# tobiashepp/torch-mednet

Hardware: AMD Instinct MI355X
Metric: 128^3 patches/sec training, 3D U-Net 32-base-ch (higher is better)
Workload: dtype bf16; 1 GPU; ResidualUNet3D f_maps=[32, 64, 128, 256] 4-class, 128^3 patches, batch 4/GPU, fwd+DiceLoss+bwd+allreduce+Adam (BASELINE config 2); global_batch=4, parallelism=dp1, graph_replay=False, gradient_exchange=none (1 rank)

## Files before the change

include/mednet_hip.h:

```cpp
#ifndef MEDNET_HIP_H
#define MEDNET_HIP_H
#include <stddef.h>
#include <stdint.h>
#ifdef __cplusplus
extern "C" {
#endif

typedef void* mednet_stream;

enum { MEDNET_F32 = 0, MEDNET_BF16 = 1,
       MEDNET_F16 = 2,
       MEDNET_U8 = 3,
       MEDNET_I64 = 4   };
enum { MEDNET_NDHWC = 0, MEDNET_NCDHW = 1 };
enum { MEDNET_ACT_NONE = 0, MEDNET_ACT_RELU = 1, MEDNET_ACT_LEAKY = 2, MEDNET_ACT_ELU = 3 };
enum { MEDNET_POOL_MAX = 0, MEDNET_POOL_AVG = 1 };
enum { MEDNET_ALGO_AUTO = 0, MEDNET_ALGO_DIRECT = 1, MEDNET_ALGO_MFMA = 2, MEDNET_ALGO_EXACT = 3,
       MEDNET_ALGO_EXACT_BIT = 4,
       MEDNET_ALGO_SPLITW_BIT = 8 };
enum { MEDNET_PACK_LOW = 0x100,
       MEDNET_PACK_HIGH_ONLY = 0x200 };
enum { MEDNET_REG_L2 = 0, MEDNET_REG_L1 = 1 };
enum { MEDNET_CLASS_DICE = 0, MEDNET_CLASS_CE = 1, MEDNET_CLASS_DICE_CE = 2 };
enum {
// ... 56 lines not shown
int mednet_conv3d_wgrad_c1_gn(const void* x, const void* dz, const void* y, const float* coef, const float* bcoef, float* dw,
                              int n, int d, int h, int w, int cout, int act, int x_dtype, int dtype, void* ws, size_t ws_bytes,
                              mednet_stream stream);
int mednet_conv3d_wgrad_cm_gn_supported(int cin, int cout, int x_dtype, int dtype);
int mednet_conv3d_wgrad_cm_plan(int n, int d, int h, int w, int cin, int cout, int dtype, int gn, int* out4);
int mednet_conv3d_wgrad_cm_gn(const void* x, int x_layout, const void* dz, const void* y, const float* coef, const float* bcoef,
                              float* dw, int n, int d, int h, int w, int cin, int cout, int act, int x_dtype, int dtype, void* ws,
                              size_t ws_bytes, mednet_stream stream);
int mednet_conv3d_wgrad(const void* x, const void* dy, float* dw, float* dbias, int n, int d, int h, int w,
                        int cin, int cout, int ksize, int x_dtype, int x_layout, int dy_dtype, int dy_layout,
                        int algo, int workgroups, void* ws, size_t ws_bytes, mednet_stream stream);

int mednet_convt3d_fwd(const void* x, const void* packed, const float* bias, const void* skip, void* y, int n,
                       int d, int h, int w, int cin, int cout, int x_dtype, int y_dtype, int algo,
                       mednet_stream stream);
int mednet_convt3d_dgrad(const void* dy, const void* packed, void* dx, int n, int d, int h, int w, int cin,
                         int cout, int dy_dtype, int dx_dtype, int algo, mednet_stream stream);
size_t mednet_convt3d_wgrad_ws_bytes(int n, int d, int h, int w, int cin, int cout, int workgroups);
int mednet_convt3d_wgrad(const void* x, const void* dy, float* dw, float* dbias, int n, int d, int h, int w,
                         int cin, int cout, int x_dtype, int dy_dtype, int algo, int workgroups, void* ws,
                         size_t ws_bytes, mednet_stream stream);

size_t mednet_gn_ws_bytes(int n, int c, size_t spatial);
int mednet_gn_stats(const void* x, const float* gamma, const float* beta, float* stats, float* coef, int n,
                    size_t spatial, int c, int groups, float eps, int dtype, void* ws, size_t ws_bytes,
                    mednet_stream stream);
int mednet_gn_finalize(const float* partial, int chunks, const float* gamma, const float* beta, float* stats,
                       float* coef, int n, size_t spatial, int c, int groups, float eps, void* ws, size_t ws_bytes,
                       mednet_stream stream);
int mednet_gn_act_fwd(const void* x, const float* coef, const void* residual, void* z, int n, size_t spatial,
// ... 253 lines not shown
```

torch-mednet_amd/csrc/api.hip:

```cpp
#include <stdarg.h>
#include <string.h>
#include "common.h"
#include "conv.h"

static thread_local char g_err[512] = "";

int mednet_internal_fail(int code, const char* fmt, ...) {
  va_list ap;
  va_start(ap, fmt);
  vsnprintf(g_err, sizeof(g_err), fmt, ap);
  va_end(ap);
  return code;
}
int mednet_internal_check_launch(const char* what) {
  const hipError_t e = hipGetLastError();
  if (e != hipSuccess) return mednet_internal_fail(MEDNET_E_HIP, "%s: %s", what, hipGetErrorString(e));
  return MEDNET_OK;
}

struct Option {
  char name[32];
  int value;
};
static Option g_options[48];
// ... 636 lines not shown
    return fail(MEDNET_E_UNSUPPORTED, "convt3d_fwd: MFMA path does not take cin=%d cout=%d", cin, cout);
  if (mfma_ok && algo_base(algo) != MEDNET_ALGO_DIRECT)
    return ELT_CALL(x_dtype, launch_convt_fwd_mfma, x, pack_mfma(packed, L, 0), bias, skip, y, n, d, h, w, cin, cout,
                    (hipStream_t)stream, algo_lo_delta(algo, x_dtype, L));
  if (f32_mode) {
    if (algo_x3(algo) && L.mfma_bytes && conv_x3_supported(cin, cout, 3))
      return launch_convt_fwd_x3(x, pack_mfma(packed, L, 0), L.lo_delta, bias, skip, y, n, d, h, w, cin, cout, (hipStream_t)stream);
    return launch_convt_fwd_f32_mfma(x, pack_f32(packed, L, 0), bias, skip, y, n, d, h, w, cin, cout, (hipStream_t)stream);
  }
  ConvGeom g;
  g.n = n; g.od = 2 * d; g.oh = 2 * h; g.ow = 2 * w; g.id = d; g.ih = h; g.iw = w;
  g.k = cin; g.m = cout; g.ks = 3; g.in_planar = 0; g.out_planar = 0;
  return launch_direct<MAP_CT_FWD>(x, pack_f32(packed, L, 0), bias, skip, y, g, x_dtype, y_dtype, (hipStream_t)stream);
}

extern "C" int mednet_convt3d_dgrad(const void* dy, const void* packed, void* dx, int n, int d, int h, int w, int cin,
                                    int cout, int dy_dtype, int dx_dtype, int algo, mednet_stream stream) {
  int rc = conv_common_checks("convt3d_dgrad", n, d, h, w, cin, cout, 3, dy_dtype, dx_dtype);
  if (rc) return rc;
  const PackLayout L = pack_layout(cin, cout, 3);
  const bool mfma_ok = L.mfma_bytes && cin % 32 == 0 && cout % 32 == 0 && is16(dy_dtype) && dx_dtype == dy_dtype &&
                       conv_mfma_fits(n, 2 * d, 2 * h, 2 * w, cout);
  const bool f32_mode = algo_f32_mode(algo, dy_dtype, dx_dtype);
  if (algo_base(algo) == MEDNET_ALGO_MFMA && !mfma_ok && !f32_mode)
    return fail(MEDNET_E_UNSUPPORTED, "convt3d_dgrad: MFMA path does not take cin=%d cout=%d", cin, cout);
  if (mfma_ok && algo_base(algo) != MEDNET_ALGO_DIRECT)
    return ELT_CALL(dy_dtype, launch_convt_dgrad_mfma, dy, pack_mfma(packed, L, 1), dx, n, d, h, w, cin, cout,
                    (hipStream_t)stream, algo_lo_delta(algo, dy_dtype, L));
  if (f32_mode) {
    if (algo_x3(algo) && L.mfma_bytes && conv_x3_supported(cin, cout, 3) && conv_x3_fits(2 * d, 2 * h, 2 * w, cout))
// ... 66 lines not shown
```

torch-mednet_amd/csrc/conv_mfma.hip:

```cpp
#include <type_traits>
#include "conv.h"

#include "elt16.inc"

namespace mednet {

template <int KIND>
struct FwdTile;
template <>
struct FwdTile<1> {
  static constexpr int TZ = 4, TY = 8, TX = 16, STRIDE = 1;
};
template <>
struct FwdTile<2> {
  static constexpr int TZ = 2, TY = 4, TX = 16, STRIDE = 2;
};
template <>
struct FwdTile<3> {
  static constexpr int TZ = 4, TY = 8, TX = 8, STRIDE = 1;
};
static bool narrow_bricks(int w) {
  const int mode = tuning_option("conv_narrow", 1);
  return mode != 0 && (w <= 8 || (mode == 2 && (w + 7) / 8 < 2 * ((w + 15) / 16)));
}
// ... 1024 lines not shown
      if (oz < od && oy < oh && ox < ow) {
        const size_t o = ((((size_t)n * od + oz) * oh + oy) * ow + ox) * a.cout + cb * 32 + piece * 8;
        const eltx8 sk = skr[it];
        eltx8 ov;
#pragma unroll
        for (int j = 0; j < 4; ++j) {
          ov[j] = (elt)(lo[j] + (float)sk[j]);
          ov[4 + j] = (elt)(hi[j] + (float)sk[4 + j]);
        }
        *reinterpret_cast<eltx8*>(a.y + o) = ov;
      }
    }
  }
}

int launch_convt_fwd_mfma(const void* x, const void* sec, const float* bias, const void* skip, void* y, int n, int d,
                          int h, int w, int cin, int cout, hipStream_t s, size_t lo_delta) {
  constexpr size_t lds = 512 * 32 * 4;
  static_assert(lds >= ((size_t)2 * 3 * 5 * 17 + 27 * 2 * 32) * 16 && lds <= 80 * 1024, "LDS plan of convt_fwd");
  CtArgs a;
  a.x = (const elt*)x;
  a.wpk = (const elt*)sec;
  a.bias = bias;
  a.skip = (const elt*)skip;
  a.y = (elt*)y;
  a.n = n; a.id = d; a.ih = h; a.iw = w; a.cin = cin; a.cout = cout;
  a.tiles_z = (d + 1) / 2;
  a.tiles_y = (h + 3) / 4;
  a.tiles_x = (w + 15) / 16;
  a.ntiles = n * a.tiles_z * a.tiles_y * a.tiles_x;
  a.nkc_in = cin / 16;
  a.nkc = lo_delta ? 2 * a.nkc_in : a.nkc_in;
// ... 412 lines not shown
  GnbSpec g;
  g.y = gn_y;
  g.z = gn_z;
  g.act = gn_act;
  return launch_fwd<2>(dy, packed_section, dx, n, d, h, w, 2 * d, 2 * h, 2 * w, cout, cin, gn_partial, s, MEDNET_ACT_NONE, nullptr, g,
                       nullptr, lo_delta);
}

struct Wg2Args {
  const elt* A;
  const elt* B;
  float* part;
  int n, d, h, w, ka, kb;
  int tiles_z, tiles_y, tiles_x, ntiles;
  int nab, nbb, splits;
  unsigned rcp_tiles_x, rcp_tiles_y, rcp_tiles_z;
  unsigned bytesA, bytesB;
};

template <int TX>
__global__ __launch_bounds__(512, 2) void wgrad_mfma2_kernel(Wg2Args a) {
  constexpr int TZ = 4, TY = 8, HZ = TZ + 2, HY = TY + 2, HX = TX + 2;
  static_assert(TX == 16 || TX == 8, "brick widths");
  constexpr int NA = TZ * TY * TX, NB = HZ * HY * HX;
  constexpr int A_ROUNDS = NA * 4 / 512, B_ROUNDS = (NB * 4 + 511) / 512;
  constexpr int KSTEPS = NA / 16;
  typedef __attribute__((ext_vector_type(4))) unsigned u32x4;
  extern __shared__ __attribute__((aligned(16))) char smem[];
  elt* A_lds = reinterpret_cast<elt*>(smem);
  elt* B_lds = reinterpret_cast<elt*>(smem) + NA * 32;
// ... 60 lines not shown
  };

  f32x16 acc[7];
#pragma unroll
  for (int i = 0; i < 7; ++i)
#pragma unroll
    for (int j = 0; j < 16; ++j) acc[i][j] = 0.f;
  const char* Ab = reinterpret_cast<const char*>(A_lds) + coloff;
  const char* Bb = reinterpret_cast<const char*>(B_lds) + coloff;
  int toff[7];
#pragma unroll
  for (int i = 0; i < 7; ++i) {
    const int tap = tw + 4 * i < 27 ? tw + 4 * i : 26;
    toff[i] = (((tap / 9) * HY + (tap / 3) % 3) * HX + tap % 3) * 64;
  }

  int tile = split;
  const int t_step = a.splits, t_end = a.ntiles;
  if (tile < t_end) {
    const Next first = plan_next(tile, true);
#pragma unroll
    for (int j = 0; j < A_ROUNDS + B_ROUNDS; ++j) fetch_one(j, first);
  }
  static_assert(A_ROUNDS + B_ROUNDS <= KSTEPS / 2, "one staging load per k-step");
  for (; tile < t_end; tile += t_step) {
    __syncthreads();
    commit();
    __syncthreads();
    const Next nx = plan_next(tile + t_step, tile + t_step < t_end);
#pragma unroll
    for (int k2 = 0; k2 < KSTEPS / 2; ++k2) {
      const int ks = 2 * k2 + kgrp;
      const eltx8 fa = tr_operand(Ab + (ks * 16 + 8 * hk + q) * 64, 4 * 64);
      const int krow = TX == 16 ? ks : 2 * ks;
      const char* brow = Bb + (((krow / TY) * HY + krow % TY) * HX + (TX == 16 ? 8 * hk : hk * HX) + q) * 64;
      eltx8 fb[7];
#pragma unroll
      for (int i = 0; i < 7; ++i) fb[i] = tr_operand(brow + toff[i], 4 * 64);
      if (k2 < A_ROUNDS + B_ROUNDS) fetch_one(k2, nx);
#pragma unroll
      for (int i = 0; i < 7; ++i) acc[i] = MEDNET_MFMA_32x32x16(fa, fb[i], acc[i], 0, 0, 0);
    }
  }
  float* mlds = reinterpret_cast<float*>(smem);
#pragma unroll
  for (int i0 = 0; i0 < 7; i0 += 4) {
    __syncthreads();
    if (kgrp == 1) {
#pragma unroll
      for (int i = i0; i < (i0 + 4 < 7 ? i0 + 4 : 7); ++i)
#pragma unroll
        for (int j = 0; j < 16; ++j) mlds[((tw * 4 + (i - i0)) * 16 + j) * 64 + lane] = acc[i][j];
    }
    __syncthreads();
    if (kgrp == 0) {
#pragma unroll
// ... 20 lines not shown
static void wgrad2_plan(int n, int d, int h, int w, int ka, int kb, int workgroups, Wg2Args& a) {
  const int tx = wgrad2_tx(w);
  a.tiles_z = (d + 3) / 4;
  a.tiles_y = (h + 7) / 8;
  a.tiles_x = (w + tx - 1) / tx;
  a.ntiles = n * a.tiles_z * a.tiles_y * a.tiles_x;
  a.rcp_tiles_x = fastdiv_rcp(a.tiles_x); a.rcp_tiles_y = fastdiv_rcp(a.tiles_y); a.rcp_tiles_z = fastdiv_rcp(a.tiles_z);
  a.nab = (ka + 31) / 32;
  a.nbb = (kb + 31) / 32;
  const int pairs = a.nab * a.nbb;
  const int target = workgroups > 0 ? workgroups : 256;
  int splits = (target + pairs - 1) / pairs;
  if (splits > a.ntiles) splits = a.ntiles;
  if (splits < 1) splits = 1;
  a.splits = splits;
}
static size_t wgrad2_ws_bytes(int n, int d, int h, int w, int cin, int cout, int workgroups) {
  Wg2Args a;
  wgrad2_plan(n, d, h, w, cout, cin, workgroups, a);
  return (size_t)a.nab * a.nbb * a.splits * 27 * 1024 * sizeof(float);
}

__global__ __launch_bounds__(256) void wgrad_mfma_reduce_kernel_few(const float* __restrict__ part, float* __restrict__ dw, int ka, int kb, int nbb,
                                               int splits) {
  __shared__ float tile[8][32 * 27 + 1];
  const int pair = (int)blockIdx.x >> 2, a0 = ((int)blockIdx.x & 3) * 8;
  const int ab = pair / nbb, bb = pair % nbb;
  const int tr = threadIdx.x >> 5, tb = threadIdx.x & 31;
  const float* src = part + ((size_t)pair * splits) * 27 * 1024 + (size_t)(a0 + tr) * 32 + tb;
#pragma unroll 3
// ... 35 lines not shown
    for (; k < splits; k += 4) s0 += src[(size_t)k * slab];
  }
  sh[threadIdx.x] = (s0 + s1) + (s2 + s3);
  __syncthreads();
  if (g == 0 && e < total && ab * 32 + a32 < ka && bb * 32 + b32 < kb)
    dw[((size_t)(ab * 32 + a32) * kb + bb * 32 + b32) * 27 + tap] = (sh[threadIdx.x] + sh[64 + threadIdx.x]) + (sh[128 + threadIdx.x] + sh[192 + threadIdx.x]);
}

struct Wg4Args {
  const elt* A;
  const elt* B;
  float* part;
  int n, d, h, w, ka, kb;
  int tiles_y, tiles_x, zslabs, zs, nitems;
  int nab, nbb, splits, xcd_remap;
  unsigned rcp_tiles_x, rcp_tiles_y, rcp_zslabs;
  unsigned bytesA, bytesB;
};

#ifndef MEDNET_WG4_DEPTH
#define MEDNET_WG4_DEPTH 3
#endif
constexpr int WG4_DEPTH = MEDNET_WG4_DEPTH;
constexpr int WG4_RB = WG4_DEPTH + 3, WG4_RA = WG4_DEPTH + 1;
constexpr int WG4_BSLOT = 12 * 1024, WG4_ASLOT = 8 * 1024;
constexpr size_t WG4_LDS = (size_t)WG4_RB * WG4_BSLOT + (size_t)WG4_RA * WG4_ASLOT;

__global__ __launch_bounds__(256, 2) void wgrad_mfma4_kernel(Wg4Args a) {
  constexpr int TY = 8, TX = 16, HX = 18;
  constexpr int D = WG4_DEPTH, RB = WG4_RB, RA = WG4_RA, BSLOT = WG4_BSLOT, ASLOT = WG4_ASLOT;
// ... 7 lines not shown
  const int g = lane >> 4, q = (lane & 15) >> 2, p = lane & 3, hk = lane >> 5;
  const int lanepart = (8 * hk + q) * 64 + (16 * (g & 1) + 4 * p) * 2;

  f32x16 acc[7];
#pragma unroll
  for (int i = 0; i < 7; ++i)
#pragma unroll
    for (int j = 0; j < 16; ++j) acc[i][j] = 0.f;
  int tap_dz[7], tap_off[7];
#pragma unroll
  for (int i = 0; i < 7; ++i) {
    const int tap = tw + 4 * i < 27 ? tw + 4 * i : 26;
    tap_dz[i] = tap / 9;
    tap_off[i] = (((tap / 3) % 3) * HX + tap % 3) * 64;
  }

  const int first = a.xcd_remap ? (split & 7) * (a.splits >> 3) + (split >> 3) : split;
  const int my_items = first < a.nitems ? (a.nitems - first + a.splits - 1) / a.splits : 0;
  const int TPI = a.zs + 2;
  const int load_ticks = my_items * TPI, total_ticks = my_items > 0 ? load_ticks + D : 0;

  int li = 0, lt = 0;
  int it_z0 = 0, it_y0 = 0;
  const elt* it_A = a.A;
  const elt* it_B = a.B;
  unsigned voffA = OOB, voffB[3] = {OOB, OOB, OOB};
  auto open_item = [&](int k) {
    int t = first + k * a.splits;
    int qd = fastdiv(t, a.tiles_x, a.rcp_tiles_x);
    const int x0 = (t - qd * a.tiles_x) * TX;
// ... 73 lines not shown
#pragma unroll
    for (int ks = 0; ks < 8; ++ks) {
      const int cur = ks & 1, nxt = cur ^ 1;
      if (ks == 7) {
        asm volatile("s_waitcnt vmcnt(%0)" ::"n"((D - 1) * 5) : "memory");
        asm volatile("s_waitcnt lgkmcnt(0)" ::: "memory");
        __builtin_amdgcn_s_barrier();
        const int nA = cA + 1 >= RA ? 0 : cA + 1, nB = cB0 + 1 >= RB ? 0 : cB0 + 1;
        if (T + 1 >= D) bases(T + 1 == D ? cA : nA, T + 1 == D ? cB0 : nB);
      }
      const int nks = ks == 7 ? 0 : ks + 1;
#pragma unroll
      for (int i = 0; i < 7; ++i) {
        __builtin_amdgcn_sched_barrier(0);
        if constexpr (COMPUTE) {
          const eltx8 fa = __builtin_shufflevector(opA[cur][0], opA[cur][1], 0, 1, 2, 3, 4, 5, 6, 7);
          const eltx8 fb = __builtin_shufflevector(opB[cur][i][0], opB[cur][i][1], 0, 1, 2, 3, 4, 5, 6, 7);
          acc[i] = MEDNET_MFMA_32x32x16(fa, fb, acc[i], 0, 0, 0);
        }
        __builtin_amdgcn_sched_barrier(0);
        constexpr int first_rd[8] = {0, 3, 6, 9, 12, 14, 16, 16};
        for (int idx = first_rd[i]; idx < first_rd[i + 1]; ++idx) rd(nxt, idx, nks);
        if (i == 6 && ks < 5) dma(ks, live);
      }
    }
  };
  if (my_items > 0) open_item(0);
  for (; T < total_ticks; ++T) {
    if (ct >= 2) tick(std::true_type{});
    else tick(std::false_type{});
    sBw = sBw + 1 >= RB ? 0 : sBw + 1;
    sAw = sAw + 1 >= RA ? 0 : sAw + 1;
    if (++lt == TPI) {
      lt = 0;
      ++li;
      if (li < my_items) open_item(li);
    }
// ... 23 lines not shown
  a.zslabs = slabs;
  a.zs = (d + slabs - 1) / slabs;
  a.tiles_y = (h + 7) / 8;
  a.tiles_x = (w + 15) / 16;
  a.nitems = n * slabs * a.tiles_y * a.tiles_x;
  a.rcp_tiles_x = fastdiv_rcp(a.tiles_x); a.rcp_tiles_y = fastdiv_rcp(a.tiles_y); a.rcp_zslabs = fastdiv_rcp(a.zslabs);
  a.nab = (ka + 31) / 32;
  a.nbb = (kb + 31) / 32;
  const int pairs = a.nab * a.nbb;
  const int target = workgroups > 0 ? workgroups : 256;
  int splits = (target + pairs - 1) / pairs;
  if (splits > a.nitems) splits = a.nitems;
  if (splits < 1) splits = 1;
  a.splits = splits;
  a.xcd_remap = splits % 8 == 0 ? 1 : 0;
}
static size_t wgrad4_ws_bytes(int n, int d, int h, int w, int cin, int cout, int workgroups) {
  Wg4Args a;
  wgrad4_plan(n, d, h, w, cout, cin, workgroups, a);
  return (size_t)a.nab * a.nbb * a.splits * 27 * 1024 * sizeof(float);
}

int wgrad_mfma_plan(int n, int d, int h, int w, int cin, int cout, int workgroups, int* out) {
  if (wgrad4_applies(d, h, w)) {
    Wg4Args a;
    wgrad4_plan(n, d, h, w, cout, cin, workgroups, a);
    const int v[10] = {4, a.nab * a.nbb * a.splits, a.nab * a.nbb, a.splits, a.nitems, a.tiles_x, a.tiles_y, a.zslabs, a.zs, a.xcd_remap};
    for (int i = 0; i < 10; ++i) out[i] = v[i];
  } else {
    Wg2Args a;
// ... 58 lines not shown
  const size_t need = wgrad_part_bytes(a);
  MEDNET_REQUIRE(ws_bytes >= need, MEDNET_E_WORKSPACE, "wgrad_mfma2: workspace %zu < %zu", ws_bytes, need);
  const int rc = launch_lds("wgrad_mfma2", tx == 8 ? wgrad_mfma2_kernel<8> : wgrad_mfma2_kernel<16>, dim3(a.nab * a.nbb * a.splits), dim3(512), lds, s, a);
  return rc ? rc : launch_wgrad_reduce(a.part, dw, cout, cin, a.nab, a.nbb, a.splits, s);
}

#include "conv_first_mfma.inc"

struct Ct2Args {
  const elt* A;
  const elt* B;
  float* part;
  int n, d, h, w, ka, kb;
  int tiles_z, tiles_y, tiles_x, ntiles;
  int nab, nbb, splits;
  unsigned rcp_tiles_x, rcp_tiles_y, rcp_tiles_z;
  unsigned bytesA, bytesB;
};

__global__ __launch_bounds__(512, 2) void convt_wgrad_mfma2_kernel(Ct2Args a) {
  constexpr int TZ = 2, TY = 4, TX = 16, HZ = TZ + 1, HY = TY + 1, HX = TX + 1;
  constexpr int NJ = TZ * TY * TX, NAH = HZ * HY * HX;
  constexpr int A_ROUNDS = (NAH * 4 + 511) / 512, B_ROUNDS = 8 * NJ * 4 / 512;
  constexpr int KSTEPS = NJ / 16;
  constexpr int A_BYTES = 16384;
  typedef __attribute__((ext_vector_type(4))) unsigned u32x4;
  extern __shared__ __attribute__((aligned(16))) char smem[];
  char* A_lds = smem;
  char* B_lds = smem + A_BYTES;

// ... 11 lines not shown
    const int t1 = tw == 0 ? 14 : tw == 1 ? 15 : tw == 2 ? 11 : 5;
    const int t2 = tw == 0 ? 16 : tw == 1 ? 21 : tw == 2 ? 19 : 7;
    const int t3 = tw == 0 ? 17 : tw == 1 ? 24 : tw == 2 ? 20 : 8;
    const int t4 = tw == 0 ? 22 : tw == 1 ? 1 : tw == 2 ? 3 : 9;
    const int t5 = tw == 0 ? 23 : tw == 1 ? 2 : tw == 2 ? 6 : 18;
    const int t6 = tw == 0 ? 25 : tw == 1 ? 0 : tw == 2 ? 26 : 18;
    const int tt[7] = {t0, t1, t2, t3, t4, t5, t6};
#pragma unroll
    for (int i = 0; i < 7; ++i) {
      const int kz = tt[i] / 9, ky = (tt[i] / 3) % 3, kx = tt[i] % 3;
      tap_of[i] = tt[i];
      boff[i] = (((kz != 1) * 4 + (ky != 1) * 2 + (kx != 1)) * NJ) * 64;
      if (i == 0 || i == 4 || i == 6) aoff[i == 0 ? 0 : i == 4 ? 1 : 2] = (((kz == 0) * HY + (ky == 0)) * HX + (kx == 0)) * 64;
    }
  }

  constexpr unsigned OOB = 0xFFFFFF00u;
  u32x4 regA[A_ROUNDS], regB[B_ROUNDS];
  struct Next {
    int tz0, ty0, tx0;
    unsigned kill;
    __amdgpu_buffer_rsrc_t rA, rB;
  };
  auto plan_next = [&](int tile, bool valid) {
    Next nx;
    int tt = valid ? tile : 0;
    int qd = fastdiv(tt, a.tiles_x, a.rcp_tiles_x);
    nx.tx0 = (tt - qd * a.tiles_x) * TX;
    tt = qd;
    qd = fastdiv(tt, a.tiles_y, a.rcp_tiles_y);
// ... 57 lines not shown
    for (int j = 0; j < A_ROUNDS + B_ROUNDS; ++j) fetch_one(j, first);
  }
  constexpr int LOADS_PER_STEP = (A_ROUNDS + B_ROUNDS + KSTEPS / 2 - 1) / (KSTEPS / 2);
  for (; tile < t_end; tile += t_step) {
    __syncthreads();
    commit();
    __syncthreads();
    const Next nx = plan_next(tile + t_step, tile + t_step < t_end);
#pragma unroll
    for (int k2 = 0; k2 < KSTEPS / 2; ++k2) {
      const int ks = 2 * k2 + kgrp;
      const char* arow = Ab + (((ks / TY) * HY + ks % TY) * HX) * 64;
      const char* brow = Bb + (ks * TX) * 64;
      eltx8 fa[3], fb[7];
#pragma unroll
      for (int i = 0; i < 3; ++i) fa[i] = tr_operand(arow + aoff[i], 4 * 64);
#pragma unroll
      for (int i = 0; i < 7; ++i) fb[i] = tr_operand(brow + boff[i], 4 * 64);
#pragma unroll
      for (int l = 0; l < LOADS_PER_STEP; ++l)
        if (k2 * LOADS_PER_STEP + l < A_ROUNDS + B_ROUNDS) fetch_one(k2 * LOADS_PER_STEP + l, nx);
#pragma unroll
      for (int i = 0; i < 7; ++i) acc[i] = MEDNET_MFMA_32x32x16(fa[i < 4 ? 0 : i < 6 ? 1 : 2], fb[i], acc[i], 0, 0, 0);
    }
  }
  float* mlds = reinterpret_cast<float*>(smem);
#pragma unroll
  for (int i0 = 0; i0 < 7; i0 += 4) {
    __syncthreads();
    if (kgrp == 1) {
#pragma unroll
      for (int i = i0; i < (i0 + 4 < 7 ? i0 + 4 : 7); ++i)
#pragma unroll
        for (int j = 0; j < 16; ++j) mlds[((tw * 4 + (i - i0)) * 16 + j) * 64 + lane] = acc[i][j];
    }
    __syncthreads();
    if (kgrp == 0) {
#pragma unroll
// ... 15 lines not shown
}

static void ct2_plan(int n, int d, int h, int w, int ka, int kb, int workgroups, Ct2Args& a) {
  a.tiles_z = (d + 1) / 2;
  a.tiles_y = (h + 3) / 4;
  a.tiles_x = (w + 15) / 16;
  a.ntiles = n * a.tiles_z * a.tiles_y * a.tiles_x;
  a.rcp_tiles_x = fastdiv_rcp(a.tiles_x); a.rcp_tiles_y = fastdiv_rcp(a.tiles_y); a.rcp_tiles_z = fastdiv_rcp(a.tiles_z);
  a.nab = (ka + 31) / 32;
  a.nbb = (kb + 31) / 32;
  const int pairs = a.nab * a.nbb;
  int splits = ((workgroups > 0 ? workgroups : 256) + pairs - 1) / pairs;
  if (splits > a.ntiles) splits = a.ntiles;
  if (splits < 1) splits = 1;
  a.splits = splits;
}

size_t convt_wgrad_mfma_ws_bytes(int n, int d, int h, int w, int cin, int cout, int workgroups) {
  if (cin % 32 || cout % 32) return 0;
  Ct2Args b;
  ct2_plan(n, d, h, w, cin, cout, workgroups, b);
  return (size_t)b.nab * b.nbb * b.splits * 27 * 1024 * sizeof(float);
}

int launch_convt_wgrad_mfma(const void* x, const void* dy, float* dw, int n, int d, int h, int w, int cin, int cout,
                            void* ws, size_t ws_bytes, hipStream_t s, int workgroups) {
  constexpr size_t lds = 16384 + 8 * 128 * 64;
  Ct2Args a;
  wgrad_operands(a, x, cin, dy, cout, 8, ws, n, d, h, w);
  ct2_plan(n, d, h, w, cin, cout, workgroups, a);
// ... 8 lines not shown
```

torch-mednet_amd/csrc/conv_mfma_decl.inc:

```
struct PackLayout {
  int taps;
  size_t f32_fwd, f32_bwd;
  size_t mfma_fwd, mfma_bwd;
  size_t mfma_bytes;
  size_t lo_delta;
  size_t total;
};
PackLayout pack_layout(int cin, int cout, int ksize);
struct PackJobDev {
  const float* w;
  void* sec_fwd;
  void* sec_bwd;
  float* Pf;
  float* Pb;
  int cin, cout, transposed;
  unsigned nblocks;
  int lo_delta;
  unsigned first_block;
};
bool conv_mfma_fits(int n, int d, int h, int w, int c);
bool conv_mfma_supported(int cin, int cout, int ksize, int x_dtype, int y_dtype, int x_layout, int y_layout, bool bias);
int launch_conv_mfma(const void* x, const void* packed_section, void* y, int n, int d, int h, int w, int cin, int cout,
                     int x_dtype, int y_dtype, float* gn_partial, hipStream_t s, int act = MEDNET_ACT_NONE,
                     const void* add = nullptr, size_t lo_delta = 0);
// ... 3 lines not shown
int conv_mfma_plan(int n, int d, int h, int w, int cin, int cout, bool gnb, int stride, int* out, bool split = false);
int conv_mfma_stats_chunks(int n, int d, int h, int w, int cin, int cout, bool gnb = false, bool split = false);
int launch_pack_mfma(const float* w, void* sec_fwd, void* sec_bwd, float* Pf, float* Pb, int cin, int cout, int T,
                     int transposed_src, hipStream_t s, size_t lo_delta = 0);
unsigned pack_mfma_blocks(int cin, int cout);
int launch_pack_mfma_many(const void* table_device, int njobs, unsigned max_blocks, hipStream_t s, int with_low = 0);
bool wgrad_mfma_supported(int cin, int cout, int ksize, int x_dtype, int dy_dtype, int x_layout, int dy_layout);
bool wgrad_mfma_fits(int n, int d, int h, int w, int cmax, int scale);
bool wgrad_mfma_coresident(int d, int h, int w);
int wgrad_mfma_plan(int n, int d, int h, int w, int cin, int cout, int workgroups, int* out);
size_t wgrad_mfma_ws_bytes(int n, int d, int h, int w, int cin, int cout, int ksize, int workgroups);
int launch_wgrad_mfma(const void* x, const void* dy, float* dw, int n, int d, int h, int w, int cin, int cout, int dtype,
                      void* ws, size_t ws_bytes, hipStream_t s, int workgroups);
int launch_convt_fwd_mfma(const void* x, const void* sec, const float* bias, const void* skip, void* y, int n, int d,
                          int h, int w, int cin, int cout, hipStream_t s, size_t lo_delta = 0);
int launch_convt_dgrad_mfma(const void* dy, const void* packed_section, void* dx, int n, int d, int h, int w, int cin,
                            int cout, hipStream_t s, size_t lo_delta = 0);
int convt_dgrad_gn_rows(int n, int d, int h, int w, int cin, int cout, bool split = false);
int launch_convt_dgrad_gn_mfma(const void* dy, const void* packed_section, void* dx, const void* gn_y, const void* gn_z, int gn_act,
                               float* gn_partial, int n, int d, int h, int w, int cin, int cout, hipStream_t s, size_t lo_delta = 0);
size_t convt_wgrad_mfma_ws_bytes(int n, int d, int h, int w, int cin, int cout, int workgroups);
int launch_convt_wgrad_mfma(const void* x, const void* dy, float* dw, int n, int d, int h, int w, int cin, int cout,
                            void* ws, size_t ws_bytes, hipStream_t s, int workgroups);

bool conv_first_mfma_supported(int cin, int cout, int ksize, int x_dtype, int y_dtype, int y_layout, bool bias);
int conv_first_stats_chunks(int n, int d, int h, int w, int cout);
int launch_conv_first_mfma(const void* x, int x_layout, int x_dtype, const float* w_pf, void* y, int n, int d, int h, int w, int cin,
                           int cout, float* gn_partial, hipStream_t s, int split = 0);
bool wgrad_first_mfma_supported(int cin, int cout, int x_dtype, int dy_dtype);
void wgrad_first_mfma_plan(int n, int d, int h, int w, int cin, int cout, bool gn, int* out4);
// ... 37 lines not shown
```

torch-mednet_amd/mednet_hip/_lib.py:

```python
from __future__ import annotations

import ctypes as C
import os

import torch

_HERE = os.path.dirname(os.path.abspath(__file__))
LIB_PATH = os.environ.get("MEDNET_LIB_PATH") or os.path.join(_HERE, "libmednet_hip.so")

F32, BF16 = 0, 1
NDHWC, NCDHW = 0, 1
ACT_NONE, ACT_RELU, ACT_LEAKY, ACT_ELU = 0, 1, 2, 3
POOL_MAX, POOL_AVG = 0, 1
ALGO_AUTO, ALGO_DIRECT, ALGO_MFMA, ALGO_EXACT = 0, 1, 2, 3
ALGO_EXACT_BIT = 4
ALGO_SPLITW_BIT = 8
PACK_LOW = 0x100
PACK_HIGH_ONLY = 0x200
REG_L2, REG_L1 = 0, 1
CLASS_DICE, CLASS_CE, CLASS_DICE_CE = 0, 1, 2
PAD_CONSTANT, PAD_SYMMETRIC = 0, 1
MIP_MEAN, MIP_MAX = 0, 1
BLEND_PROBABILITIES, BLEND_LOGITS = 0, 1
INTERP_LINEAR, INTERP_NEAREST = 0, 1
# ... 36 lines not shown
    "mednet_pool2_bwd_gn_rows": (_i, [_i] * 6),
    "mednet_convt3d_dgrad_gn_rows": (_i, [_i] * 8),
    "mednet_convt3d_dgrad_gn": (_i, [_vp] * 5 + [_i, _vp] + [_i] * 8 + [_vp]),
    "mednet_pool2_bwd_gn": (_i, [_vp] * 5 + [_i, _vp] + [_i] * 7 + [_vp]),
    "mednet_conv3d_wgrad_ws_bytes": (_sz, [_i] * 8),
    "mednet_conv3d_wgrad_coresident": (_i, [_i] * 10),
    "mednet_conv3d_wgrad_plan": (_i, [_i] * 8 + [_vp]),
    "mednet_conv3d_wgrad_c1_gn_supported": (_i, [_i] * 3),
    "mednet_conv3d_wgrad_c1_gn": (_i, [_vp] * 6 + [_i] * 8 + [_vp, _sz, _vp]),
    "mednet_conv3d_cm_supported": (_i, [_i] * 6),
    "mednet_conv3d_wgrad_cm_gn_supported": (_i, [_i] * 4),
    "mednet_conv3d_wgrad_cm_plan": (_i, [_i] * 8 + [_vp]),
    "mednet_conv3d_wgrad_cm_gn": (_i, [_vp, _i] + [_vp] * 5 + [_i] * 9 + [_vp, _sz, _vp]),
    "mednet_conv3d_wgrad": (_i, [_vp, _vp, _vp, _vp] + [_i] * 13 + [_vp, _sz, _vp]),
    "mednet_convt3d_fwd": (_i, [_vp, _vp, _vp, _vp, _vp] + [_i] * 9 + [_vp]),
    "mednet_convt3d_dgrad": (_i, [_vp, _vp, _vp] + [_i] * 9 + [_vp]),
    "mednet_convt3d_wgrad_ws_bytes": (_sz, [_i] * 7),
    "mednet_convt3d_wgrad": (_i, [_vp, _vp, _vp, _vp] + [_i] * 10 + [_vp, _sz, _vp]),
    "mednet_gn_ws_bytes": (_sz, [_i, _i, _sz]),
    "mednet_gn_stats": (_i, [_vp, _vp, _vp, _vp, _vp, _i, _sz, _i, _i, _f, _i, _vp, _sz, _vp]),
    "mednet_gn_act_fwd": (_i, [_vp, _vp, _vp, _vp, _i, _sz, _i, _i, _i, _i, _vp]),
    "mednet_gn_act_bwd": (_i, [_vp] * 11 + [_i, _sz, _i, _i, _i, _i, _i, _vp, _sz, _vp]),
    "mednet_act_fwd": (_i, [_vp, _vp, _sz, _i, _i, _vp]),
    "mednet_act_bwd": (_i, [_vp, _vp, _vp, _sz, _i, _i, _vp]),
    "mednet_add": (_i, [_vp, _vp, _vp, _sz, _i, _vp]),
    "mednet_pool2_fwd": (_i, [_vp, _vp] + [_i] * 7 + [_vp]),
    "mednet_bn_stats": (_i, [_vp] * 6 + [_f, _vp, _vp, _i, _sz, _i, _f, _i, _vp, _sz, _vp]),
    "mednet_bn_eval_coef": (_i, [_vp] * 6 + [_i, _i, _f, _vp]),
    "mednet_bn_act_bwd": (_i, [_vp] * 10 + [_i, _sz, _i, _i, _i, _i, _i, _vp, _sz, _vp]),
    "mednet_bn_act_bwd_fused": (_i, [_vp] * 6 + [_i, _vp, _vp, _vp, _i, _sz, _i, _i, _i, _i, _i, _vp, _sz, _vp]),
# ... 159 lines not shown
```

Before: 207.9 patches/s.

## Add persistent register-resident-weight transposed-conv forward kernel and skip duplicate wgrad MFMA

Adds a specialized persistent MFMA kernel for the 64->32 channel transposed 3D convolution forward. It keeps all packed weights in registers, splits the eight output parity classes across four waves, double-buffers the input halo in LDS with XCD-aware tile ordering, and fuses bias and skip-add into a swizzled LDS epilogue. Separately, the wgrad kernels skip the redundant seventh MFMA and its operand reads on the wave whose last tap slot duplicates tap 26. The special kernel is gated on a 256-CU device and enough tiles, and adds a plan query API. The cost is register pressure at one block per CU plus more code paths to validate.

```diff
diff --git a/include/mednet_hip.h b/include/mednet_hip.h
--- a/include/mednet_hip.h
+++ b/include/mednet_hip.h
@@ -94,6 +94,7 @@
 int mednet_convt3d_fwd(const void* x, const void* packed, const float* bias, const void* skip, void* y, int n,
                        int d, int h, int w, int cin, int cout, int x_dtype, int y_dtype, int algo,
                        mednet_stream stream);
+int mednet_convt3d_fwd_plan(int n, int d, int h, int w, int cin, int cout, int dtype, int algo, int* out4);
 int mednet_convt3d_dgrad(const void* dy, const void* packed, void* dx, int n, int d, int h, int w, int cin,
                          int cout, int dy_dtype, int dx_dtype, int algo, mednet_stream stream);
 size_t mednet_convt3d_wgrad_ws_bytes(int n, int d, int h, int w, int cin, int cout, int workgroups);
diff --git a/torch-mednet_amd/csrc/api.hip b/torch-mednet_amd/csrc/api.hip
--- a/torch-mednet_amd/csrc/api.hip
+++ b/torch-mednet_amd/csrc/api.hip
@@ -674,6 +674,13 @@
   return launch_direct<MAP_CT_FWD>(x, pack_f32(packed, L, 0), bias, skip, y, g, x_dtype, y_dtype, (hipStream_t)stream);
 }
 
+extern "C" int mednet_convt3d_fwd_plan(int n, int d, int h, int w, int cin, int cout, int dtype, int algo, int* out4) {
+  MEDNET_REQUIRE(out4 && n > 0 && d > 0 && h > 0 && w > 0, MEDNET_E_SHAPE, "convt3d_fwd_plan: bad arguments");
+  MEDNET_REQUIRE(is16(dtype) && cin % 32 == 0 && cout % 32 == 0 && algo_base(algo) != MEDNET_ALGO_DIRECT, MEDNET_E_UNSUPPORTED,
+                 "convt3d_fwd_plan: the 16-bit matrix-core kernels only (dtype %d, %d -> %d, algo %d)", dtype, cin, cout, algo);
+  return ELT_CALL(dtype, convt_fwd_mfma_plan, n, d, h, w, cin, cout, algo_split(algo, dtype), out4);
+}
+
 extern "C" int mednet_convt3d_dgrad(const void* dy, const void* packed, void* dx, int n, int d, int h, int w, int cin,
                                     int cout, int dy_dtype, int dx_dtype, int algo, mednet_stream stream) {
   int rc = conv_common_checks("convt3d_dgrad", n, d, h, w, cin, cout, 3, dy_dtype, dx_dtype);
diff --git a/torch-mednet_amd/csrc/conv_mfma.hip b/torch-mednet_amd/csrc/conv_mfma.hip
--- a/torch-mednet_amd/csrc/conv_mfma.hip
+++ b/torch-mednet_amd/csrc/conv_mfma.hip
@@ -1062,8 +1062,36 @@
   }
 }
 
+#include "convt_fwd32_mfma.inc"
+
+static bool convt_fwd32_takes(int n, int d, int h, int w, int cin, int cout, bool split) {
+  const long long ntiles = (long long)n * ((d + 1) / 2) * ((h + 3) / 4) * ((w + 15) / 16);
+  return cin == 64 && cout == 32 && !split && ntiles >= 256 && ntiles < (1ll << 31) && conv_mfma_fits(n, 2 * d, 2 * h, 2 * w, cout) &&
+         ::mednet_internal_cu_count() == 256 && tuning_option("convt_fwd32", 1);
+}
+int convt_fwd_mfma_plan(int n, int d, int h, int w, int cin, int cout, bool split, int* out) {
+  const int ntiles = n * ((d + 1) / 2) * ((h + 3) / 4) * ((w + 15) / 16);
+  const bool special = convt_fwd32_takes(n, d, h, w, cin, cout, split);
+  out[0] = special ? 2 : 1;
+  out[1] = special ? 256 : (ntiles + 7) / 8 * 8 * (cout / 32);
+  out[2] = ntiles;
+  out[3] = special && ntiles % 8 == 0 ? ntiles / 8 : 0;
+  return MEDNET_OK;
+}
+
 int launch_convt_fwd_mfma(const void* x, const void* sec, const float* bias, const void* skip, void* y, int n, int d,
                           int h, int w, int cin, int cout, hipStream_t s, size_t lo_delta) {
+  if (convt_fwd32_takes(n, d, h, w, cin, cout, lo_delta != 0)) {
+    Cf32Args c;
+    c.x = (const elt*)x; c.wpk = (const elt*)sec; c.bias = bias; c.skip = (const elt*)skip; c.y = (elt*)y;
+    c.n = n; c.id = d; c.ih = h; c.iw = w;
+    c.tiles_z = (d + 1) / 2; c.tiles_y = (h + 3) / 4; c.tiles_x = (w + 15) / 16;
+    c.ntiles = n * c.tiles_z * c.tiles_y * c.tiles_x;
+    c.rcp_tiles_x = fastdiv_rcp(c.tiles_x); c.rcp_tiles_y = fastdiv_rcp(c.tiles_y); c.rcp_tiles_z = fastdiv_rcp(c.tiles_z);
+    c.bytes_x = (unsigned)((size_t)d * h * w * 64 * 2);
+    c.bytes_y = (unsigned)((size_t)8 * d * h * w * 32 * 2);
+    return launch_lds("convt_fwd32_mfma", convt_fwd32_mfma_kernel, dim3(256), dim3(256), CF32_LDS, s, c);
+  }
   constexpr size_t lds = 512 * 32 * 4;
   static_assert(lds >= ((size_t)2 * 3 * 5 * 17 + 27 * 2 * 32) * 16 && lds <= 80 * 1024, "LDS plan of convt_fwd");
   CtArgs a;
@@ -1506,6 +1534,7 @@
   int n, d, h, w, ka, kb;
   int tiles_z, tiles_y, tiles_x, ntiles;
   int nab, nbb, splits;
+  int skip_dup;
   unsigned rcp_tiles_x, rcp_tiles_y, rcp_tiles_z;
   unsigned bytesA, bytesB;
 };
@@ -1596,6 +1625,7 @@
     const int tap = tw + 4 * i < 27 ? tw + 4 * i : 26;
     toff[i] = (((tap / 9) * HY + (tap / 3) % 3) * HX + tap % 3) * 64;
   }
+  const bool dup6 = a.skip_dup != 0 && tw == 3;
 
   int tile = split;
   const int t_step = a.splits, t_end = a.ntiles;
@@ -1621,7 +1651,8 @@
       for (int i = 0; i < 7; ++i) fb[i] = tr_operand(brow + toff[i], 4 * 64);
       if (k2 < A_ROUNDS + B_ROUNDS) fetch_one(k2, nx);
 #pragma unroll
-      for (int i = 0; i < 7; ++i) acc[i] = MEDNET_MFMA_32x32x16(fa, fb[i], acc[i], 0, 0, 0);
+      for (int i = 0; i < 7; ++i)
+        if (!(i == 6 && dup6)) acc[i] = MEDNET_MFMA_32x32x16(fa, fb[i], acc[i], 0, 0, 0);
     }
   }
   float* mlds = reinterpret_cast<float*>(smem);
@@ -1672,6 +1703,7 @@
   if (splits > a.ntiles) splits = a.ntiles;
   if (splits < 1) splits = 1;
   a.splits = splits;
+  a.skip_dup = tuning_option("wgrad_skip_dup", 1);
 }
 static size_t wgrad2_ws_bytes(int n, int d, int h, int w, int cin, int cout, int workgroups) {
   Wg2Args a;
@@ -1737,6 +1769,7 @@
   int n, d, h, w, ka, kb;
   int tiles_y, tiles_x, zslabs, zs, nitems;
   int nab, nbb, splits, xcd_remap;
+  int skip_dup;
   unsigned rcp_tiles_x, rcp_tiles_y, rcp_zslabs;
   unsigned bytesA, bytesB;
 };
@@ -1774,6 +1807,7 @@
     tap_dz[i] = tap / 9;
     tap_off[i] = (((tap / 3) % 3) * HX + tap % 3) * 64;
   }
+  const bool dup6 = a.skip_dup != 0 && tw == 3;
 
   const int first = a.xcd_remap ? (split & 7) * (a.splits >> 3) + (split >> 3) : split;
   const int my_items = first < a.nitems ? (a.nitems - first + a.splits - 1) / a.splits : 0;
@@ -1877,13 +1911,16 @@
       for (int i = 0; i < 7; ++i) {
         __builtin_amdgcn_sched_barrier(0);
         if constexpr (COMPUTE) {
-          const eltx8 fa = __builtin_shufflevector(opA[cur][0], opA[cur][1], 0, 1, 2, 3, 4, 5, 6, 7);
-          const eltx8 fb = __builtin_shufflevector(opB[cur][i][0], opB[cur][i][1], 0, 1, 2, 3, 4, 5, 6, 7);
-          acc[i] = MEDNET_MFMA_32x32x16(fa, fb, acc[i], 0, 0, 0);
+          if (!(i == 6 && dup6)) {
+            const eltx8 fa = __builtin_shufflevector(opA[cur][0], opA[cur][1], 0, 1, 2, 3, 4, 5, 6, 7);
+            const eltx8 fb = __builtin_shufflevector(opB[cur][i][0], opB[cur][i][1], 0, 1, 2, 3, 4, 5, 6, 7);
+            acc[i] = MEDNET_MFMA_32x32x16(fa, fb, acc[i], 0, 0, 0);
+          }
         }
         __builtin_amdgcn_sched_barrier(0);
         constexpr int first_rd[8] = {0, 3, 6, 9, 12, 14, 16, 16};
-        for (int idx = first_rd[i]; idx < first_rd[i + 1]; ++idx) rd(nxt, idx, nks);
+        for (int idx = first_rd[i]; idx < first_rd[i + 1]; ++idx)
+          if (!(idx >= 14 && dup6)) rd(nxt, idx, nks);
         if (i == 6 && ks < 5) dma(ks, live);
       }
     }
@@ -1937,6 +1974,7 @@
   if (splits < 1) splits = 1;
   a.splits = splits;
   a.xcd_remap = splits % 8 == 0 ? 1 : 0;
+  a.skip_dup = tuning_option("wgrad_skip_dup", 1);
 }
 static size_t wgrad4_ws_bytes(int n, int d, int h, int w, int cin, int cout, int workgroups) {
   Wg4Args a;
@@ -2025,6 +2063,7 @@
   int n, d, h, w, ka, kb;
   int tiles_z, tiles_y, tiles_x, ntiles;
   int nab, nbb, splits;
+  int skip_dup;
   unsigned rcp_tiles_x, rcp_tiles_y, rcp_tiles_z;
   unsigned bytesA, bytesB;
 };
@@ -2066,6 +2105,8 @@
       if (i == 0 || i == 4 || i == 6) aoff[i == 0 ? 0 : i == 4 ? 1 : 2] = (((kz == 0) * HY + (ky == 0)) * HX + (kx == 0)) * 64;
     }
   }
+
+  const bool dup6 = a.skip_dup != 0 && tw == 3;
 
   constexpr unsigned OOB = 0xFFFFFF00u;
   u32x4 regA[A_ROUNDS], regB[B_ROUNDS];
@@ -2153,14 +2194,17 @@
       const char* brow = Bb + (ks * TX) * 64;
       eltx8 fa[3], fb[7];
 #pragma unroll
-      for (int i = 0; i < 3; ++i) fa[i] = tr_operand(arow + aoff[i], 4 * 64);
-#pragma unroll
-      for (int i = 0; i < 7; ++i) fb[i] = tr_operand(brow + boff[i], 4 * 64);
+      for (int i = 0; i < 3; ++i)
+        if (!(i == 2 && dup6)) fa[i] = tr_operand(arow + aoff[i], 4 * 64);
+#pragma unroll
+      for (int i = 0; i < 7; ++i)
+        if (!(i == 6 && dup6)) fb[i] = tr_operand(brow + boff[i], 4 * 64);
 #pragma unroll
       for (int l = 0; l < LOADS_PER_STEP; ++l)
         if (k2 * LOADS_PER_STEP + l < A_ROUNDS + B_ROUNDS) fetch_one(k2 * LOADS_PER_STEP + l, nx);
 #pragma unroll
-      for (int i = 0; i < 7; ++i) acc[i] = MEDNET_MFMA_32x32x16(fa[i < 4 ? 0 : i < 6 ? 1 : 2], fb[i], acc[i], 0, 0, 0);
+      for (int i = 0; i < 7; ++i)
+        if (!(i == 6 && dup6)) acc[i] = MEDNET_MFMA_32x32x16(fa[i < 4 ? 0 : i < 6 ? 1 : 2], fb[i], acc[i], 0, 0, 0);
     }
   }
   float* mlds = reinterpret_cast<float*>(smem);
@@ -2206,6 +2250,7 @@
   if (splits > a.ntiles) splits = a.ntiles;
   if (splits < 1) splits = 1;
   a.splits = splits;
+  a.skip_dup = tuning_option("wgrad_skip_dup", 1);
 }
 
 size_t convt_wgrad_mfma_ws_bytes(int n, int d, int h, int w, int cin, int cout, int workgroups) {
diff --git a/torch-mednet_amd/csrc/conv_mfma_decl.inc b/torch-mednet_amd/csrc/conv_mfma_decl.inc
--- a/torch-mednet_amd/csrc/conv_mfma_decl.inc
+++ b/torch-mednet_amd/csrc/conv_mfma_decl.inc
@@ -41,6 +41,7 @@
                       void* ws, size_t ws_bytes, hipStream_t s, int workgroups);
 int launch_convt_fwd_mfma(const void* x, const void* sec, const float* bias, const void* skip, void* y, int n, int d,
                           int h, int w, int cin, int cout, hipStream_t s, size_t lo_delta = 0);
+int convt_fwd_mfma_plan(int n, int d, int h, int w, int cin, int cout, bool split, int* out4);
 int launch_convt_dgrad_mfma(const void* dy, const void* packed_section, void* dx, int n, int d, int h, int w, int cin,
                             int cout, hipStream_t s, size_t lo_delta = 0);
 int convt_dgrad_gn_rows(int n, int d, int h, int w, int cin, int cout, bool split = false);
diff --git a/torch-mednet_amd/csrc/convt_fwd32_mfma.inc b/torch-mednet_amd/csrc/convt_fwd32_mfma.inc
--- /dev/null
+++ b/torch-mednet_amd/csrc/convt_fwd32_mfma.inc
@@ -0,0 +1,232 @@
+constexpr int CF32_NV = 3 * 5 * 17;
+constexpr int CF32_IMG_SLOTS = 8 * CF32_NV;
+constexpr int CF32_EPI_SLOT0 = 2 * CF32_IMG_SLOTS;
+constexpr size_t CF32_LDS = (size_t)(CF32_EPI_SLOT0 + 4 * 256 + 64) * 16;
+
+__host__ __device__ constexpr int cf32_ncls(int w) { return w == 0 ? 1 : w == 1 ? 3 : 2; }
+__host__ __device__ constexpr int cf32_cls(int w, int pos) {
+  return w == 0 ? 7 : w == 1 ? (pos == 0 ? 3 : pos == 1 ? 1 : 0) : w == 2 ? (pos == 0 ? 5 : 2) : (pos == 0 ? 6 : 4);
+}
+__host__ __device__ constexpr int cf32_ntaps(int cls) { return (1 + ((cls >> 2) & 1)) * (1 + ((cls >> 1) & 1)) * (1 + (cls & 1)); }
+__host__ __device__ constexpr int cf32_tap(int cls, int i) {
+  const int pz = (cls >> 2) & 1, py = (cls >> 1) & 1, px = cls & 1;
+  const int ix = i % (1 + px), iy = (i / (1 + px)) % (1 + py), iz = i / ((1 + px) * (1 + py));
+  return (pz ? 2 * iz : 1) * 9 + (py ? 2 * iy : 1) * 3 + (px ? 2 * ix : 1);
+}
+__host__ __device__ constexpr int cf32_first(int w, int pos) {
+  int s = 0;
+  for (int p = 0; p < pos; ++p) s += cf32_ntaps(cf32_cls(w, p));
+  return s;
+}
+static_assert(cf32_first(0, 1) == 8 && cf32_first(1, 3) == 7 && cf32_first(2, 2) == 6 && cf32_first(3, 2) == 6, "27 taps over the four waves");
+static_assert(cf32_tap(7, 0) == 0 && cf32_tap(7, 7) == 26 && cf32_tap(0, 0) == 13 && cf32_tap(3, 1) == 11 && cf32_tap(4, 1) == 22, "tap order of a class");
+
+__device__ __forceinline__ void cf32_mfma_zero(f32x16& acc, const eltx8& w_in_agpr, const eltx8& b) {
+  asm volatile(MEDNET_MFMA_ASM_OP " %0, %1, %2, 0" : "=&v"(acc) : "a"(w_in_agpr), "v"(b));
+}
+
+struct Cf32Args {
+  const elt* x;
+  const elt* wpk;
+  const float* bias;
+  const elt* skip;
+  elt* y;
+  int n, id, ih, iw;
+  int tiles_z, tiles_y, tiles_x, ntiles;
+  unsigned rcp_tiles_x, rcp_tiles_y, rcp_tiles_z;
+  unsigned bytes_x, bytes_y;
+};
+
+template <int W>
+__device__ __forceinline__ void convt_fwd32_wave(const Cf32Args& a, char* smem) {
+  constexpr int TZ = 2, TY = 4, TX = 16, HY = 5, HX = 17, NV = CF32_NV;
+  constexpr int NCLS = cf32_ncls(W), NT = cf32_first(W, NCLS);
+  constexpr int IN_ROUNDS = 8;
+  constexpr unsigned OOB = 0xFFFFFF00u;
+  typedef __attribute__((ext_vector_type(4))) unsigned u32x4;
+  u32x4* img = reinterpret_cast<u32x4*>(smem);
+  f32x4* epi = reinterpret_cast<f32x4*>(smem) + CF32_EPI_SLOT0 + W * 256;
+  const int tid = threadIdx.x, lane = tid & 63;
+  const int r = lane & 31, h = lane >> 5;
+  const int spare_slot = CF32_EPI_SLOT0 + 4 * 256 + lane;
+
+  eltx8 wreg[4 * NT];
+  {
+    const u32x4* wp = reinterpret_cast<const u32x4*>(a.wpk) + h * 32 + r;
+#pragma unroll
+    for (int pos = 0; pos < NCLS; ++pos)
+#pragma unroll
+      for (int kc = 0; kc < 4; ++kc)
+#pragma unroll
+        for (int ti = 0; ti < cf32_ntaps(cf32_cls(W, pos)); ++ti)
+          wreg[kc * NT + cf32_first(W, pos) + ti] = __builtin_bit_cast(eltx8, wp[(kc * 27 + cf32_tap(cf32_cls(W, pos), ti)) * 64]);
+  }
+  float bv[16];
+#pragma unroll
+  for (int q = 0; q < 4; ++q)
+#pragma unroll
+    for (int j = 0; j < 4; ++j) bv[q * 4 + j] = a.bias ? a.bias[8 * q + 4 * h + j] : 0.f;
+
+  auto origin = [&](int tile, int& n, int& tz0, int& ty0, int& tx0) {
+    int tt = tile;
+    int qd = fastdiv(tt, a.tiles_x, a.rcp_tiles_x);
+    tx0 = (tt - qd * a.tiles_x) * TX;
+    tt = qd;
+    qd = fastdiv(tt, a.tiles_y, a.rcp_tiles_y);
+    ty0 = (tt - qd * a.tiles_y) * TY;
+    tt = qd;
+    qd = fastdiv(tt, a.tiles_z, a.rcp_tiles_z);
+    tz0 = (tt - qd * a.tiles_z) * TZ;
+    n = qd;
+  };
+  const int xcd_chunk = a.ntiles % 8 == 0 ? a.ntiles / 8 : 0;
+  const int seq_step = xcd_chunk ? (int)(gridDim.x >> 3) : (int)gridDim.x;
+  const int seq_end = xcd_chunk ? xcd_chunk : a.ntiles;
+  int seq = xcd_chunk ? (int)(blockIdx.x >> 3) : (int)blockIdx.x;
+  auto tile_of = [&](int q) { return xcd_chunk ? (int)(blockIdx.x & 7) * xcd_chunk + q : q; };
+  if (seq >= seq_end) return;
+
+  u32x4 in_reg[IN_ROUNDS];
+  auto load_round = [&](int it, int n, int tz0, int ty0, int tx0, bool valid) {
+    const int p = it * 256 + tid, v = p >> 3, piece = p & 7;
+    const int hx = v % HX, hy = (v / HX) % HY, hz = v / (HX * HY);
+    const bool ok = (v < NV) & (tz0 + hz < a.id) & (ty0 + hy < a.ih) & (tx0 + hx < a.iw);
+    const unsigned voff = ok ? (unsigned)((hz * a.ih + hy) * a.iw + hx) * 128u + (unsigned)piece * 16u : OOB;
+    const unsigned soff = (unsigned)((tz0 * a.ih + ty0) * a.iw + tx0) * 128u;
+    const elt* base = a.x + (size_t)n * a.id * a.ih * a.iw * 64;
+    in_reg[it] = __builtin_amdgcn_raw_buffer_load_b128(__builtin_amdgcn_make_buffer_rsrc((void*)base, 0, a.bytes_x & (0u - (unsigned)valid), 0x00020000),
+                                                       voff, soff, 0);
+  };
+  auto commit = [&](int buf) {
+#pragma unroll
+    for (int it = 0; it < IN_ROUNDS; ++it) {
+      const int p = it * 256 + tid, v = p >> 3, piece = p & 7;
+      img[v < NV ? buf * CF32_IMG_SLOTS + piece * NV + v : spare_slot] = in_reg[it];
+    }
+  };
+
+  const int lx = ((r & 15) - (r >> 4) * HX) & 15;
+  int lbase[4];
+#pragma unroll
+  for (int t = 0; t < 4; ++t) lbase[t] = h * NV + ((t >> 1) * HY + 2 * (t & 1) + (r >> 4)) * HX + lx;
+  const int ev = lane >> 2, pj = lane & 3;
+  const int key_w = ((lx >> 1) & 3) | ((lx & 1) << 2), key_r = ((ev >> 1) & 3) | ((ev & 1) << 2);
+  const int vl = (r >> 4) * 16 + lx;
+  const int od = 2 * a.id, oh = 2 * a.ih, ow = 2 * a.iw;
+  (void)od;
+
+  {
+    int n0, tz0, ty0, tx0;
+    origin(tile_of(seq), n0, tz0, ty0, tx0);
+#pragma unroll
+    for (int it = 0; it < IN_ROUNDS; ++it) load_round(it, n0, tz0, ty0, tx0, true);
+    commit(0);
+  }
+  int cur = 0;
+  while (true) {
+    int n, tz0, ty0, tx0;
+    origin(tile_of(seq), n, tz0, ty0, tx0);
+    const bool has_next = seq + seq_step < seq_end;
+    int n2, tz2, ty2, tx2;
+    origin(tile_of(has_next ? seq + seq_step : seq), n2, tz2, ty2, tx2);
+    __syncthreads();
+    const u32x4* im = img + cur * CF32_IMG_SLOTS;
+
+    const size_t ysample = (size_t)n * a.bytes_y;
+    const __amdgpu_buffer_rsrc_t y_rsrc = __builtin_amdgcn_make_buffer_rsrc((void*)(reinterpret_cast<char*>(a.y) + ysample), 0, a.bytes_y, 0x00020000);
+    const __amdgpu_buffer_rsrc_t skip_rsrc =
+        __builtin_amdgcn_make_buffer_rsrc((void*)(reinterpret_cast<const char*>(a.skip) + ysample), 0, a.skip ? a.bytes_y : 0u, 0x00020000);
+    const unsigned lane_voff = tx0 + ev < a.iw ? (unsigned)(ev * 128 + pj * 16) : OOB;
+    auto row_voff = [&](int t, int j) { return ((tz0 + (t >> 1) < a.id) & (ty0 + 2 * (t & 1) + j < a.ih)) ? lane_voff : OOB; };
+    auto row_soff = [&](int cls, int t, int j) {
+      const int oz = 2 * (tz0 + (t >> 1)) + ((cls >> 2) & 1), oy = 2 * (ty0 + 2 * (t & 1) + j) + ((cls >> 1) & 1), ox = 2 * tx0 + (cls & 1);
+      return (unsigned)((oz * oh + oy) * ow + ox) * 64u;
+    };
+
+    auto do_class = [&](auto pos_tag) {
+      constexpr int POS = decltype(pos_tag)::value, CLS = cf32_cls(W, POS), NTAP = cf32_ntaps(CLS), FIRST = cf32_first(W, POS);
+      constexpr int STEPS = 4 * NTAP;
+      eltx8 skr[8];
+#pragma unroll
+      for (int t = 0; t < 4; ++t)
+#pragma unroll
+        for (int j = 0; j < 2; ++j)
+          skr[t * 2 + j] = __builtin_bit_cast(eltx8, __builtin_amdgcn_raw_buffer_load_b128(skip_rsrc, row_voff(t, j), row_soff(CLS, t, j), 0));
+      auto b_operand = [&](int s, int t) {
+        const int kc = s / NTAP, tap = cf32_tap(CLS, s % NTAP);
+        const int dz = tap / 9 == 0, dy = (tap / 3) % 3 == 0, dx = tap % 3 == 0;
+        return __builtin_bit_cast(eltx8, im[lbase[t] + 2 * kc * NV + (dz * HY + dy) * HX + dx]);
+      };
+      f32x16 acc[4];
+      eltx8 xb[2][4];
+#pragma unroll
+      for (int t = 0; t < 4; ++t) xb[0][t] = b_operand(0, t);
+#pragma unroll
+      for (int s = 0; s < STEPS; ++s) {
+        const int kc = s / NTAP, ti = s % NTAP;
+        __builtin_amdgcn_sched_barrier(0);
+        if (s + 1 < STEPS) {
+#pragma unroll
+          for (int t = 0; t < 4; ++t) xb[(s + 1) & 1][t] = b_operand(s + 1, t);
+        }
+        if (POS == 0 && (ti == 0 || ti == 2)) load_round(kc * 2 + (ti >> 1), n2, tz2, ty2, tx2, has_next);
+        __builtin_amdgcn_sched_barrier(0);
+#pragma unroll
+        for (int t = 0; t < 4; ++t) {
+          if (s == 0) cf32_mfma_zero(acc[t], wreg[kc * NT + FIRST + ti], xb[s & 1][t]);
+          else mfma_a_acc(acc[t], wreg[kc * NT + FIRST + ti], xb[s & 1][t]);
+        }
+      }
+      asm volatile("s_nop 15\n\ts_nop 7" : "+v"(acc[0]), "+v"(acc[1]), "+v"(acc[2]), "+v"(acc[3]));
+      __builtin_amdgcn_sched_barrier(0);
+
+#pragma unroll
+      for (int t = 0; t < 4; ++t) {
+        wave_lds_fence();
+#pragma unroll
+        for (int q = 0; q < 4; ++q) {
+          f32x4 o;
+#pragma unroll
+          for (int j = 0; j < 4; ++j) o[j] = acc[t][q * 4 + j] + bv[q * 4 + j];
+          epi[vl * 8 + ((2 * q + h) ^ key_w)] = o;
+        }
+        wave_lds_fence();
+        f32x4 lo[2], hi[2];
+#pragma unroll
+        for (int j = 0; j < 2; ++j) {
+          lo[j] = epi[(j * 16 + ev) * 8 + ((2 * pj) ^ key_r)];
+          hi[j] = epi[(j * 16 + ev) * 8 + ((2 * pj + 1) ^ key_r)];
+        }
+#pragma unroll
+        for (int j = 0; j < 2; ++j) {
+          const eltx8 sk = skr[t * 2 + j];
+          eltx8 ov;
+#pragma unroll
+          for (int k = 0; k < 4; ++k) {
+            ov[k] = (elt)(lo[j][k] + (float)sk[k]);
+            ov[4 + k] = (elt)(hi[j][k] + (float)sk[4 + k]);
+          }
+          __builtin_amdgcn_raw_buffer_store_b128(__builtin_bit_cast(u32x4, ov), y_rsrc, row_voff(t, j), row_soff(CLS, t, j), 0);
+        }
+      }
+    };
+    do_class(std::integral_constant<int, 0>{});
+    if constexpr (NCLS > 1) do_class(std::integral_constant<int, 1>{});
+    if constexpr (NCLS > 2) do_class(std::integral_constant<int, 2>{});
+
+    if (!has_next) break;
+    commit(cur ^ 1);
+    seq += seq_step;
+    cur ^= 1;
+  }
+}
+
+__global__ __launch_bounds__(256, 1) void convt_fwd32_mfma_kernel(Cf32Args a) {
+  extern __shared__ __attribute__((aligned(16))) char smem[];
+  switch (__builtin_amdgcn_readfirstlane(threadIdx.x >> 6)) {
+    case 0: convt_fwd32_wave<0>(a, smem); break;
+    case 1: convt_fwd32_wave<1>(a, smem); break;
+    case 2: convt_fwd32_wave<2>(a, smem); break;
+    default: convt_fwd32_wave<3>(a, smem); break;
+  }
+}
diff --git a/torch-mednet_amd/mednet_hip/_lib.py b/torch-mednet_amd/mednet_hip/_lib.py
--- a/torch-mednet_amd/mednet_hip/_lib.py
+++ b/torch-mednet_amd/mednet_hip/_lib.py
@@ -74,6 +74,7 @@
     "mednet_conv3d_wgrad_cm_gn": (_i, [_vp, _i] + [_vp] * 5 + [_i] * 9 + [_vp, _sz, _vp]),
     "mednet_conv3d_wgrad": (_i, [_vp, _vp, _vp, _vp] + [_i] * 13 + [_vp, _sz, _vp]),
     "mednet_convt3d_fwd": (_i, [_vp, _vp, _vp, _vp, _vp] + [_i] * 9 + [_vp]),
+    "mednet_convt3d_fwd_plan": (_i, [_i] * 8 + [_vp]),
     "mednet_convt3d_dgrad": (_i, [_vp, _vp, _vp] + [_i] * 9 + [_vp]),
     "mednet_convt3d_wgrad_ws_bytes": (_sz, [_i] * 7),
     "mednet_convt3d_wgrad": (_i, [_vp, _vp, _vp, _vp] + [_i] * 10 + [_vp, _sz, _vp]),
```

Result: no change. 206.5 patches/s (-0.6%).
